# Martinsos/edlib

Measured on AMD Instinct MI355X. Metric: GCUPS (cell updates/s), 1M x 150bp HW reads vs 5Mb target, higher is better.
Workload: dtype u32

## Files before the change

edlib_amd/csrc/engine.hpp:

```cpp
#pragma once
#include "../../include/edlib_amd.h"
#include "common.hpp"
#include "pair_kernels.hpp"
#include "lanepair.hpp"
#include "reads_kernels.hpp"
#include "cross_kernels.hpp"
#include "window_kernels.hpp"
#include "strands.hpp"
#include "flat_pairs_prepare.hpp"
#include "pairs_gather.hpp"

#include <chrono>
#include <deque>
#include <functional>
#include <memory>
#include <vector>

namespace edlib_amd {

struct Tables {
    uint8_t tlut[256];
    uint8_t idToByte[256];
    int sigmaT = 0;
    uint32_t presence[8];
// ... 155 lines not shown
    std::vector<EdlibEqualityPair> eqs_;
    int device_ = 0;
    bool shared_ = false;
    bool pairsKind_ = false;
    bool noPairs_ = false;
    int noResults(const char* who);
    int n_ = 0;
    std::vector<long long> qoff_, toff_;
    bool strands_ = false;
    PinBuf h_strand_;
    int outN() const { return strands_ ? n_ / 2 : n_; }
    int unitOf(int u) const { return strands_ ? 2 * u + h_strand_.p[u] : u; }
    void setStrand(int read, int code) { h_strand_.p[read] = (uint8_t)(code & kStrandReverse); h_strand_.p[outN() + read] = (code & kStrandBoth) ? 1 : 0; }
    int resolveStrandsOnHost(std::vector<UnitResult>& res);
    int hostStrandCounts_[4] = {0, 0, 0, 0};
    int strandCounts(int counts[4]);
    Tables tab_;
    hipStream_t stream_ = nullptr;
    Event evRun0_, evRun1_, evA_, evB_;

    DevBuf<uint8_t> d_in_;
    PinBuf h_in_;
    DevBuf<uint8_t> d_qpool_, d_tpool_, d_tlut_, d_idToByte_, d_eq8_;
    DevBuf<uint16_t> d_eqtbl_;
    hipError_t uploadEq8();
    DevBuf<uint32_t> d_presence_;
    DevBuf<long long> d_qoff_, d_toff_;

    std::vector<int> emptyUnits_, readUnits_, pairUnits_;
    std::vector<int> longUnits_;
    std::vector<int> pairNow_;
    int beginRun(hipError_t guardStatus);
    int enqueueWordSteps();
    int endRun();
    void resetRecords(std::vector<UnitResult>& res);
    void answerEmptyUnits(std::vector<UnitResult>& res);
    int runFlatPhase(std::vector<UnitResult>& res, Lap& lap);
    int runLongReads(std::vector<UnitResult>& res, Lap& lap);
    int runPairPhase(std::vector<UnitResult>& res, Lap& lap);
    int runStartsPhase(std::vector<UnitResult>& res, Lap& lap);
    int runPathsPhase(std::vector<UnitResult>& res, Lap& lap);
    void startStats();
    bool flatDone_ = false;

    struct ReadGroup {
        int nwords = 0, nslots = 0, numSegments = 1, segLen = 0, warm = 0, mMin = 0, mMax = 0;
        std::vector<int> perm;
        DevBuf<int> d_perm, d_qlen, d_kinit, d_alphaExtra, d_segBest, d_segCnt, d_segPos;
        DevBuf<int> d_best, d_total, d_pos, d_flags;
        DevBuf<uint32_t> d_peq;
        bool zeroCopy = false; PinBuf hostOut;
        std::vector<int> ovfSlots; std::vector<long long> ovfOff; DevBuf<int> d_ovfPool;
        DevBuf<int> d_lvMap, d_lvBest, d_lvCnt, d_lvPos; std::vector<int> lvMap; int lvS = 0, lvCap = 0; bool lvValid = false;
        DevBuf<int> d_list;
        int nreal = -1;
        bool mates = false; DevBuf<int> d_win;
    };
    static constexpr int kLastLevelCap = 16;
    int listOpenSlots(ReadGroup& g, int kDone, std::vector<int>& out);
    DevBuf<uint8_t> d_selTmp_;
    std::vector<std::unique_ptr<ReadGroup>> groups_;
    DevBuf<uint32_t> d_tpk_, d_trows_;
    DevBuf<unsigned long long> d_wordSteps_;
    PinBuf h_wordSteps_; bool wordStepsPending_ = false;
    DevBuf<unsigned long long> d_ringSteps_; PinBuf h_ringSteps_; bool ringStepsUsed_ = false;
    unsigned long long* ringStepsCounter();
    bool banded_ = false;
    int syms_ = 4;
    int packTarget();
    int runReads();
    int makeGroup(const std::vector<int>& units, int words, std::unique_ptr<ReadGroup>& g, long long oneRoundWaves = 0);
    int runGroupScans(ReadGroup& g, bool fullOnly);
    int runGroupExact(ReadGroup& g);
    int collectGroup(ReadGroup& g, std::vector<UnitResult>& res);
    int seedThreshold(const ReadGroup& g, bool fullOnly) const;
    int buildSeedIndex();
    int runSeedPass(ReadGroup& g, int k);
    DevBuf<uint32_t> d_seedCnt_, d_seedOff_, d_seedPos_;
    DevBuf<uint8_t> d_seedTmp_;
    bool hits_ = false, hitsHaveRun_ = false;
    HitListBuffers hitList_;
    HitRows hostHits_;
    DevBuf<int> d_hitSlotUnit_;
    DevBuf<long long> d_hitTotal_;
    int runReadHits();
    int scanGroupHits(ReadGroup& g, int slotBase);
    int hitsScanBanded(ReadGroup& g, int slotBase, const int* d_slotmap, int nlanes, int numSegments, int segLen, int warm);
    struct Piece { long long off; int len; int thr; };
    int scanPieces(const std::vector<Piece>& pieces, bool filter, std::vector<std::pair<int, int>>* cand,
                   std::vector<uint8_t>* overflow, std::vector<int>* best);
    int solveLongReads(std::vector<UnitResult>& res, std::vector<int>& fallback);
    bool filterScan_ = false;
    struct ChainArgs { const uint32_t* in = nullptr; uint32_t* out = nullptr; const int* src = nullptr; int inLanes = 0, blocks = 0; const int* rowBase = nullptr; };
    ChainArgs chain_;
    int solveTallFull(const std::vector<int>& units, std::vector<UnitResult>& res, std::vector<int>& handBack);
    int collectReads(std::vector<UnitResult>& res);
    bool readsCollected_ = true;
    int scanGroup(ReadGroup& g, int mode, const int* d_slotmap, int nlanes, int kcap, const int* d_kinit,
                  int numSegments, int segLen, int warm, int* segBest, int* segCnt, int* segPos, int cap,
                  const long long* posOff, const int* posCap, bool unbanded = false,
                  unsigned long long* wordSteps = nullptr, const uint32_t* peqDense = nullptr,
                  const int* qlenDense = nullptr, int peqBottom = 0, int* liveBest = nullptr,
                  const Segment* segTable = nullptr, long long tableCols = 0);

    DevBuf<PairDesc> d_descs_;
    DevBuf<unsigned long long> d_peq64_;
// ... 201 lines not shown
```

edlib_amd/csrc/engine_reads.hip:

```cpp
#include "engine.hpp"

#include <algorithm>
#include <chrono>
#include <cmath>
#include <condition_variable>
#include <cstring>
#include <mutex>
#include <thread>

namespace edlib_amd {

__global__ void __launch_bounds__(256)
seed_thresholds_kernel(int* __restrict__ kinit, const int* __restrict__ best, const int* __restrict__ cnt, int n)
{
    const int i = blockIdx.x * blockDim.x + threadIdx.x;
    if (i < n && cnt[i] > 0 && best[i] < kinit[i]) kinit[i] = best[i];
}


int Batch::scanGroup(ReadGroup& g, int mode, const int* d_slotmap, int nlanes, int kcap, const int* d_kinit,
                     int numSegments, int segLen, int warm, int* segBest, int* segCnt, int* segPos, int cap,
                     const long long* posOff, const int* posCap, bool unbanded, unsigned long long* wordSteps,
                     const uint32_t* peqDense, const int* qlenDense, int peqBottom, int* liveBest,
                     const Segment* segTable, long long tableCols)
{
    ReadScanArgs a{};
    a.peq = peqDense ? peqDense : g.d_peq.p; a.tpk = d_tpk_.p; a.trows = d_trows_.p; a.targetLength = tlen(0);
    if (mode == EDLIB_MODE_SHW) a.targetLength = (int)std::min<long long>(a.targetLength, 64LL * g.nwords + 1);
    a.qlen = qlenDense ? qlenDense : g.d_qlen.p; a.kinit = d_kinit; a.slotmap = d_slotmap; a.nlanes = nlanes;
    a.numSegments = numSegments; a.segLen = segLen; a.warm = warm;
    a.segBest = segBest; a.segCnt = segCnt; a.segPos = segPos; a.cap = cap;
    a.posOff = posOff; a.posCap = posCap;
    a.kcap = kcap; a.wordSteps = wordSteps ? wordSteps : d_wordSteps_.p;
    a.filter = filterScan_ ? 1 : 0;
    a.liveBest = liveBest;
    a.segTable = segTable;
    a.bottomAligned = peqBottom;
    a.chainIn = chain_.in; a.chainOut = chain_.out; a.chainSrc = chain_.src; a.chainInLanes = chain_.inLanes;
    a.chainBlocks = chain_.blocks; a.rowBase = chain_.rowBase;
    const bool chained = chain_.in != nullptr || chain_.out != nullptr;
    const bool longGroup = g.nwords > kMaxReadWords;
    const bool fullHeight = banded_ && mode == EDLIB_MODE_HW && unbanded && (chained || syms_ > 4 || longGroup);
    const bool bandedKernel = !fullHeight && banded_ && mode == EDLIB_MODE_HW && (!unbanded || syms_ > 4 || longGroup);
    static const bool dbg = getenv("EDLIB_AMD_DEBUG") != nullptr;
    if (dbg) {
        EDLIB_AMD_HIP(hipStreamSynchronize(stream_));
        fprintf(stderr, "[edlib_amd] scanGroup nwords=%d mode=%d nlanes=%d S=%d segLen=%d warm=%d cap=%d kcap=%d slotmap=%p posOff=%p rows=%s kernel=%s syms=%d\n",
                g.nwords, mode, nlanes, numSegments, segLen, warm, cap, kcap, (const void*)d_slotmap, (const void*)posOff,
                peqBottom > 1 ? "delay" : (peqBottom ? "bottom" : "top"),
                fullHeight ? "full" : (bandedKernel ? "banded" : "plain"), syms_);
        if (peqBottom > 1) fprintf(stderr, "[edlib_amd] scanGroup delayRows=%d\n", peqBottom - 1);
    }
    scanTimerStart();
    const long long colsScanned = segTable ? tableCols
        : std::min<long long>(a.targetLength, (long long)numSegments * segLen) + (long long)(numSegments - 1) * warm;
#ifdef EDLIB_AMD_DRAIN_DIAG
    const char* drainOut = (peqBottom && liveBest) ? "edlib_amd_drain.bin" : nullptr;
    DevBuf<unsigned long long> d_clk;
    const size_t drainGX = ((size_t)(nlanes + 63) / 64 + 3) / 4, drainWaves = drainGX * numSegments * 4;
    if (drainOut) {
        EDLIB_AMD_HIP(d_clk.alloc(2 * drainWaves));
        EDLIB_AMD_HIP(hipMemsetAsync(d_clk.p, 0, 2 * drainWaves * sizeof(unsigned long long), stream_));
        a.waveClock = d_clk.p;
    }
#endif
    if (peqBottom && (fullHeight || bandedKernel)) EDLIB_AMD_HIP(hipErrorInvalidValue);
    if (fullHeight) {
        EDLIB_AMD_HIP(launch_scan_reads_full(g.nwords, syms_, a, stream_));
        stats.word_steps += (long long)((nlanes + 63) / 64 * 64) * g.nwords * colsScanned;
// ... 131 lines not shown
        }
        if (resolved > 0) {
            int acc = 0, kq = kFirstMax;
            for (int d = 0; d <= kFirstMax; ++d) { acc += hist[d]; if (acc * 1000LL >= resolved * 995LL) { kq = d; break; } }
            kFirst = std::max(4, std::min(kFirstMax, kq));
        }
        if (real > 0 && resolved * 10 < real * 3) twoPass = false;
        if (twoPass && (int)open.size() * 10 > real && open.size() >= 32 && price_ladder(open, open.size(), real)) return 1;
    }
    std::vector<int> todo;
    bool haveTodo = false;
    if (kSeed >= 0) {
        if (runSeedPass(g, kFirst)) return 1;
        if (twoPass) {
            if (listOpenSlots(g, kFirst, todo)) return 1;
            haveTodo = true;
            if (g.nreal < 0) { g.nreal = 0; for (int u : g.perm) g.nreal += u >= 0; }
            if (g.nslots >= 16384 && todo.size() * 10 > (size_t)g.nreal && todo.size() >= 32) {
                const size_t nsm = std::min<size_t>(2048, todo.size());
                std::vector<int> sample(nsm);
                for (size_t i = 0; i < nsm; ++i) sample[i] = todo[i * todo.size() / nsm];
                if (price_ladder(sample, todo.size(), g.nreal)) return 1;
            }
        }
    } else {
        if (scanGroup(g, mode, nullptr, g.nslots, twoPass ? kFirst : kNoCap, g.d_kinit.p, g.numSegments, g.segLen,
                      g.warm, g.d_segBest.p, g.d_segCnt.p, g.d_segPos.p, 8, nullptr, nullptr, fullOnly)) return 1;
        const bool chained = chain_.in != nullptr || chain_.out != nullptr;
        EDLIB_AMD_HIP(launch_merge_segments(g.d_segBest.p, g.d_segCnt.p, g.d_segPos.p, g.numSegments, 8,
                                            g.nslots, nullptr, 16, g.d_best.p, g.d_total.p, g.d_pos.p,
                                            g.d_flags.p, stream_, chained ? kOvfRescan : kOvfGatherGroup));
    }
    ladder.push_back(kNoCap);
    int kDone = kFirst;
    for (size_t lv = 0; twoPass && lv < ladder.size(); ++lv) {
        const int kcapL = ladder[lv];
        const bool last = kcapL == kNoCap;
        if (!haveTodo && listOpenSlots(g, kDone, todo)) return 1;
        haveTodo = false;
        if (todo.empty()) break;
        {
            const size_t no = todo.size();
            int S2, segLen2, warm2;
            plan_segments((int)no, T, mode, g.warm, 65536, S2, segLen2, warm2);
            const int capL = last ? kLastLevelCap : 8;
            EDLIB_AMD_HIP(g.d_lvMap.ensure(no));
            int* d_map = g.d_lvMap.p;
            EDLIB_AMD_HIP(hipMemcpyAsync(d_map, todo.data(), no * sizeof(int), hipMemcpyHostToDevice, stream_));
            bool plain = false;
            if (last && no >= 4096) {
                const int np2 = 64;
                std::vector<int> sub(np2);
                for (int i = 0; i < np2; ++i) sub[i] = todo[(size_t)((long long)i * no / np2)];
                int S3, segLen3, warm3;
                plan_segments(np2, T, mode, g.warm, 16384, S3, segLen3, warm3);
                const size_t it3 = (size_t)np2 * S3;
                DevBuf<int> d_m3, d_b3, d_c3, d_p3; DevBuf<unsigned long long> d_ws;
                EDLIB_AMD_HIP(d_m3.alloc(np2)); EDLIB_AMD_HIP(d_b3.alloc(it3)); EDLIB_AMD_HIP(d_c3.alloc(it3));
                EDLIB_AMD_HIP(d_p3.alloc(it3 * 8)); EDLIB_AMD_HIP(d_ws.alloc(1));
                EDLIB_AMD_HIP(hipMemcpyAsync(d_m3.p, sub.data(), np2 * sizeof(int), hipMemcpyHostToDevice, stream_));
                EDLIB_AMD_HIP(hipMemsetAsync(d_ws.p, 0, sizeof(unsigned long long), stream_));
                if (scanGroup(g, mode, d_m3.p, np2, kNoCap, g.d_kinit.p, S3, segLen3, warm3,
                              d_b3.p, d_c3.p, d_p3.p, 8, nullptr, nullptr, false, d_ws.p)) return 1;
                unsigned long long ws = 0;
                EDLIB_AMD_HIP(hipMemcpyAsync(&ws, d_ws.p, sizeof ws, hipMemcpyDeviceToHost, stream_));
                EDLIB_AMD_HIP(hipStreamSynchronize(stream_));
                const double cols = (double)np2 * ((double)T + (double)(S3 - 1) * warm3);
                plain = (double)ws >= 0.85 * g.nwords * cols;
                stats.word_steps += (long long)ws;
            }
            const bool bottomOk = plain && mode == EDLIB_MODE_HW && syms_ == 4 && g.nwords <= kMaxReadWords &&
                                  chain_.in == nullptr && chain_.out == nullptr;
            const int bottom = !bottomOk ? 0 : 1 + delay_rows_for(g.nwords, g.mMax);
            std::vector<Segment> table;
            DevBuf<Segment> d_segTable; long long tableCols = 0;
            if (bottom && S2 > 1 && no >= 4096) {
                int resident = 0;
                EDLIB_AMD_HIP(scan_reads_resident_workgroups(g.nwords, bottom, &resident));
#ifdef EDLIB_AMD_DRAIN_UNIFORM
                resident = 0;
#endif
                table = plan_segments_tapered(T, (int)(((no + 63) / 64 + 3) / 4), resident, warm2, segLen2);
                S2 = (int)table.size();
                for (const Segment& sg : table) tableCols += sg.cols + std::min(warm2, sg.start);
                EDLIB_AMD_HIP(d_segTable.alloc(table.size()));
                EDLIB_AMD_HIP(hipMemcpyAsync(d_segTable.p, table.data(), table.size() * sizeof(Segment), hipMemcpyHostToDevice, stream_));
            }
            const size_t items = no * (size_t)S2;
            EDLIB_AMD_HIP(g.d_lvBest.ensure(items)); EDLIB_AMD_HIP(g.d_lvCnt.ensure(items));
            EDLIB_AMD_HIP(g.d_lvPos.ensure(items * capL));
            int *d_sb = g.d_lvBest.p, *d_sc = g.d_lvCnt.p, *d_sp = g.d_lvPos.p;
            const size_t no64 = (no + 63) / 64 * 64;
            std::vector<int> perm2(no64, -1);
            for (size_t i = 0; i < no; ++i) perm2[i] = g.perm[todo[i]];
            DevBuf<int> d_perm2, d_qlen2, d_kinit2, d_extra2; DevBuf<uint32_t> d_peq2;
            EDLIB_AMD_HIP(d_perm2.alloc(no64)); EDLIB_AMD_HIP(d_qlen2.alloc(no64)); EDLIB_AMD_HIP(d_kinit2.alloc(no64));
            EDLIB_AMD_HIP(d_extra2.alloc(no64)); EDLIB_AMD_HIP(d_peq2.alloc(no64 * (size_t)syms_ * g.nwords));
            EDLIB_AMD_HIP(hipMemcpyAsync(d_perm2.p, perm2.data(), no64 * sizeof(int), hipMemcpyHostToDevice, stream_));
            EDLIB_AMD_HIP(launch_build_peq_reads(g.nwords, syms_, d_qpool_.p, d_qoff_.p, d_perm2.p, (int)no64,
                                                 d_eqtbl_.p, d_presence_.p, cfg_.k, d_peq2.p, d_qlen2.p,
                                                 d_kinit2.p, d_extra2.p, stream_, bottom));
            const int seedCols = 4096;
            DevBuf<int> d_b0, d_c0, d_p0;
            if (mode == EDLIB_MODE_HW && last && no >= 4096 && S2 > 1 && T >= 16 * seedCols) {
                EDLIB_AMD_HIP(d_b0.alloc(no)); EDLIB_AMD_HIP(d_c0.alloc(no)); EDLIB_AMD_HIP(d_p0.alloc(no * 8));
                if (scanGroup(g, mode, nullptr, (int)no, kcapL, d_kinit2.p, 1, seedCols, 0,
                              d_b0.p, d_c0.p, d_p0.p, 8, nullptr, nullptr, plain, nullptr, d_peq2.p, d_qlen2.p, bottom)) return 1;
                hipLaunchKernelGGL(seed_thresholds_kernel, dim3((unsigned)((no + 255) / 256)), dim3(256), 0, stream_,
                                   d_kinit2.p, d_b0.p, d_c0.p, (int)no);
                EDLIB_AMD_HIP(hipGetLastError());
            }
            DevBuf<int> d_live2;
            if (bottom && S2 > 1) {
                EDLIB_AMD_HIP(d_live2.alloc(no64));
                EDLIB_AMD_HIP(hipMemcpyAsync(d_live2.p, d_kinit2.p, no64 * sizeof(int), hipMemcpyDeviceToDevice, stream_));
            }
            if (scanGroup(g, mode, nullptr, (int)no, kcapL, d_kinit2.p, S2, segLen2, warm2,
                          d_sb, d_sc, d_sp, capL, nullptr, nullptr, plain, nullptr, d_peq2.p, d_qlen2.p, bottom, d_live2.p,
                          d_segTable.p, tableCols)) return 1;
            EDLIB_AMD_HIP(launch_merge_segments(d_sb, d_sc, d_sp, S2, capL, (int)no, d_map, 16,
                                                g.d_best.p, g.d_total.p, g.d_pos.p, g.d_flags.p, stream_,
                                                last ? kOvfGatherLevel : kOvfRescan));
            EDLIB_AMD_HIP(hipStreamSynchronize(stream_));
            if (last) { g.lvValid = true; g.lvS = S2; g.lvCap = capL; g.lvMap.swap(todo); }
            if (dbgLadder) fprintf(stderr, "[edlib_amd] level kcap=%d: %zu slots rescanned (plain=%d)\n", kcapL, no, (int)plain);
        }
        kDone = kcapL;
    }
    return 0;
}

int Batch::listOpenSlots(ReadGroup& g, int kDone, std::vector<int>& out)
{
    size_t tmp = 0;
    EDLIB_AMD_HIP(select_slots_scratch_bytes(g.nslots, &tmp));
    EDLIB_AMD_HIP(d_selTmp_.ensure(tmp));
    EDLIB_AMD_HIP(g.d_list.ensure((size_t)g.nslots + 1));
    int* count = g.d_list.p + g.nslots;
    EDLIB_AMD_HIP(launch_select_open_slots(g.d_perm.p, g.d_total.p, g.d_qlen.p, cfg_.k, kDone, g.nslots, g.d_list.p, count,
                                           d_selTmp_.p, d_selTmp_.bytes(), stream_, g.mates));
    int n = 0;
    EDLIB_AMD_HIP(hipMemcpyAsync(&n, count, sizeof(int), hipMemcpyDeviceToHost, stream_));
    EDLIB_AMD_HIP(hipStreamSynchronize(stream_));
    out.resize((size_t)n);
    if (n > 0) {
        EDLIB_AMD_HIP(hipMemcpyAsync(out.data(), g.d_list.p, (size_t)n * sizeof(int), hipMemcpyDeviceToHost, stream_));
        EDLIB_AMD_HIP(hipStreamSynchronize(stream_));
    }
    return 0;
}


int Batch::seedThreshold(const ReadGroup& g, bool fullOnly) const
{
    const long long T = tlen(0);
    if (fullOnly || !banded_ || cfg_.mode != EDLIB_MODE_HW || syms_ != 4 || cfg_.additionalEqualitiesLength > 0 ||
        g.nwords > kMaxReadWords || chain_.in != nullptr || chain_.out != nullptr)
        return -1;
    if (T < 64LL * 32 * g.nwords || g.nslots < 1024 || (long long)g.nslots * T < (1LL << 30)) return -1;
    int kf = -1;
    for (int k = 16; k >= 0 && kf < 0; --k) {
        const int L = g.mMin / (k + 1);
        if (L >= kSeedQ && (double)(k + 1) * (double)T <= std::ldexp(1.0, 2 * L) / 8.0) kf = k;
    }
    return (kf >= 0 && kf >= std::min(8, cfg_.k >= 0 ? cfg_.k : 8)) ? kf : -1;
}

int Batch::buildSeedIndex()
{
    const int T = tlen(0);
    EDLIB_AMD_HIP(d_seedCnt_.ensure((size_t)kSeedBuckets + 1));
    EDLIB_AMD_HIP(d_seedOff_.ensure((size_t)kSeedBuckets + 1));
    EDLIB_AMD_HIP(d_seedPos_.ensure((size_t)T));
    size_t tmp = 0;
    EDLIB_AMD_HIP(seed_index_scratch_bytes(&tmp));
    EDLIB_AMD_HIP(d_seedTmp_.ensure(tmp));
    scanTimerStart();
// ... 24 lines not shown
    static const bool dbg = getenv("EDLIB_AMD_DEBUG") != nullptr;
    if (dbg) fprintf(stderr, "[edlib_amd] seed pass nwords=%d k=%d: %d of %d slots handed back\n", g.nwords, k, nb, g.nslots);
    if (nb <= 0) return 0;
    int S2, segLen2, warm2;
    plan_segments(nb, T, EDLIB_MODE_HW, g.warm, 65536, S2, segLen2, warm2);
    const size_t items = (size_t)nb * S2;
    DevBuf<int> d_sb, d_sc, d_sp;
    EDLIB_AMD_HIP(d_sb.alloc(items)); EDLIB_AMD_HIP(d_sc.alloc(items)); EDLIB_AMD_HIP(d_sp.alloc(items * 8));
    if (scanGroup(g, EDLIB_MODE_HW, d_back.p, nb, k, g.d_kinit.p, S2, segLen2, warm2, d_sb.p, d_sc.p, d_sp.p, 8,
                  nullptr, nullptr)) return 1;
    EDLIB_AMD_HIP(launch_merge_segments(d_sb.p, d_sc.p, d_sp.p, S2, 8, nb, d_back.p, 16, g.d_best.p, g.d_total.p,
                                        g.d_pos.p, g.d_flags.p, stream_));
    EDLIB_AMD_HIP(hipStreamSynchronize(stream_));
    return 0;
}

int Batch::runGroupExact(ReadGroup& g)
{
    const int T = tlen(0);
    const int mode = (cfg_.mode == EDLIB_MODE_HW || cfg_.mode == EDLIB_MODE_SHW) ? (int)cfg_.mode : (int)EDLIB_MODE_NW;
    const int kNoCap = 0x3fffffff;
    const size_t ns = (size_t)g.nslots;
    g.ovfSlots.clear(); g.ovfOff.assign(1, 0);
    if (mode == EDLIB_MODE_NW) return 0;
    std::vector<int> recs;
    if (g.zeroCopy && !g.mates) {
        EDLIB_AMD_HIP(hipStreamSynchronize(stream_));
        for (size_t s = 0; s < ns; ++s)
            if (g.d_flags.p[s] && g.perm[s] >= 0) { recs.push_back((int)s); recs.push_back(g.d_flags.p[s]); recs.push_back(g.d_total.p[s]); }
    } else {
        size_t tmp = 0;
        EDLIB_AMD_HIP(select_slots_scratch_bytes(g.nslots, &tmp));
        EDLIB_AMD_HIP(d_selTmp_.ensure(tmp));
        EDLIB_AMD_HIP(g.d_list.ensure(ns + 1));
        int* count = g.d_list.p + ns;
        EDLIB_AMD_HIP(launch_select_flagged_slots(g.d_perm.p, g.d_flags.p, g.nslots, g.d_list.p, count,
                                                  d_selTmp_.p, d_selTmp_.bytes(), stream_, g.mates ? g.d_win.p : nullptr));
        int novf = 0;
        EDLIB_AMD_HIP(hipMemcpyAsync(&novf, count, sizeof(int), hipMemcpyDeviceToHost, stream_));
        EDLIB_AMD_HIP(hipStreamSynchronize(stream_));
        if (novf > 0) {
            DevBuf<int> d_recs;
            EDLIB_AMD_HIP(d_recs.alloc((size_t)novf * 3));
            EDLIB_AMD_HIP(launch_pick_slot_records(g.d_list.p, novf, g.d_flags.p, g.d_total.p, d_recs.p, stream_));
            recs.resize((size_t)novf * 3);
            EDLIB_AMD_HIP(hipMemcpyAsync(recs.data(), d_recs.p, recs.size() * sizeof(int), hipMemcpyDeviceToHost, stream_));
            EDLIB_AMD_HIP(hipStreamSynchronize(stream_));
        }
    }
    const size_t no = recs.size() / 3;
    if (!no) return 0;
    std::vector<int> src(no, 0), at(no, -1);
    std::vector<int> rescan;
    for (size_t i = 0; i < no; ++i) {
        const int s = recs[3 * i], f = recs[3 * i + 1];
        g.ovfSlots.push_back(s);
        if (f == kOvfGatherLevel && g.lvValid) {
            const auto it = std::lower_bound(g.lvMap.begin(), g.lvMap.end(), s);
            if (it != g.lvMap.end() && *it == s) { src[i] = 1; at[i] = (int)(it - g.lvMap.begin()); }
        } else if (f == kOvfGatherGroup) { src[i] = 2; at[i] = s; }
        if (!src[i]) { at[i] = (int)rescan.size(); rescan.push_back(s); }
    }
    const size_t nr = rescan.size();
    int S2 = 1, segLen2 = 0, warm2 = 0;
    DevBuf<int> d_map, d_caps, d_sb, d_sc; DevBuf<long long> d_off;
    std::vector<int> cnts;
    if (nr) {
        plan_segments((int)nr, T, mode, g.warm, 16384, S2, segLen2, warm2, nr <= 256 ? 1024 : 4096);
        const size_t items = nr * (size_t)S2;
        EDLIB_AMD_HIP(d_map.alloc(nr)); EDLIB_AMD_HIP(d_sb.alloc(items)); EDLIB_AMD_HIP(d_sc.alloc(items));
        EDLIB_AMD_HIP(hipMemcpyAsync(d_map.p, rescan.data(), nr * sizeof(int), hipMemcpyHostToDevice, stream_));
        if (scanGroup(g, mode, d_map.p, (int)nr, kNoCap, g.d_best.p, S2, segLen2, warm2,
                      d_sb.p, d_sc.p, d_sb.p , 0, nullptr, nullptr)) return 1;
        cnts.resize(items);
        EDLIB_AMD_HIP(hipMemcpyAsync(cnts.data(), d_sc.p, items * sizeof(int), hipMemcpyDeviceToHost, stream_));
        EDLIB_AMD_HIP(hipStreamSynchronize(stream_));
    }
    std::vector<long long> offs(nr * (size_t)S2);
    std::vector<int> gIdx[2], gLim[2]; std::vector<long long> gOff[2];
    long long acc = 0;
    g.ovfOff.assign(no + 1, 0);
    for (size_t i = 0; i < no; ++i) {
        if (src[i]) {
            const int w = src[i] - 1, n = std::max(0, recs[3 * i + 2]);
            gIdx[w].push_back(at[i]); gOff[w].push_back(acc); gLim[w].push_back(n);
            acc += n;
        } else {
            const size_t r = (size_t)at[i];
            for (int sg = 0; sg < S2; ++sg) { offs[r * S2 + sg] = acc; acc += cnts[r * S2 + sg]; }
        }
        g.ovfOff[i + 1] = acc;
    }
    EDLIB_AMD_HIP(g.d_ovfPool.ensure((size_t)std::max<long long>(acc, 1)));
    DevBuf<int> d_gi[2], d_gl[2]; DevBuf<long long> d_go[2];
    for (int w = 0; w < 2; ++w) {
        const size_t n = gIdx[w].size();
        if (!n) continue;
        EDLIB_AMD_HIP(d_gi[w].alloc(n)); EDLIB_AMD_HIP(d_gl[w].alloc(n)); EDLIB_AMD_HIP(d_go[w].alloc(n));
        EDLIB_AMD_HIP(hipMemcpyAsync(d_gi[w].p, gIdx[w].data(), n * sizeof(int), hipMemcpyHostToDevice, stream_));
        EDLIB_AMD_HIP(hipMemcpyAsync(d_gl[w].p, gLim[w].data(), n * sizeof(int), hipMemcpyHostToDevice, stream_));
        EDLIB_AMD_HIP(hipMemcpyAsync(d_go[w].p, gOff[w].data(), n * sizeof(long long), hipMemcpyHostToDevice, stream_));
        if (w == 0)
            EDLIB_AMD_HIP(launch_gather_segments(g.d_lvBest.p, g.d_lvCnt.p, g.d_lvPos.p, g.lvS, g.lvCap, (int)n,
                                                 d_gi[w].p, d_go[w].p, d_gl[w].p, g.d_ovfPool.p, stream_));
        else
            EDLIB_AMD_HIP(launch_gather_segments(g.d_segBest.p, g.d_segCnt.p, g.d_segPos.p, g.numSegments, 8, (int)n,
                                                 d_gi[w].p, d_go[w].p, d_gl[w].p, g.d_ovfPool.p, stream_));
    }
    if (nr) {
        const size_t items = nr * (size_t)S2;
        EDLIB_AMD_HIP(d_caps.alloc(items)); EDLIB_AMD_HIP(d_off.alloc(items));
        EDLIB_AMD_HIP(hipMemcpyAsync(d_caps.p, cnts.data(), items * sizeof(int), hipMemcpyHostToDevice, stream_));
        EDLIB_AMD_HIP(hipMemcpyAsync(d_off.p, offs.data(), items * sizeof(long long), hipMemcpyHostToDevice, stream_));
        if (scanGroup(g, mode, d_map.p, (int)nr, kNoCap, g.d_best.p, S2, segLen2, warm2,
                      d_sb.p, d_sc.p, g.d_ovfPool.p, 0, d_off.p, d_caps.p)) return 1;
    }
    EDLIB_AMD_HIP(hipStreamSynchronize(stream_));
    static const bool dbg = getenv("EDLIB_AMD_DEBUG") != nullptr;
    if (dbg) fprintf(stderr, "[edlib_amd] exact pass nwords=%d: %zu gathered, %zu rescanned\n", g.nwords, no - nr, nr);
    stats.overflow_units += (int)no;
    return 0;
}


int Batch::hitsScanBanded(ReadGroup& g, int slotBase, const int* d_slotmap, int nlanes, int numSegments, int segLen, int warm)
{
    ReadScanArgs a{};
    a.peq = g.d_peq.p; a.tpk = d_tpk_.p; a.trows = d_trows_.p; a.targetLength = tlen(0);
    a.qlen = g.d_qlen.p; a.kinit = g.d_kinit.p; a.slotmap = d_slotmap; a.nlanes = nlanes;
    a.numSegments = numSegments; a.segLen = segLen; a.warm = warm;
    a.cap = 1;
    a.kcap = 0x3fffffff; a.wordSteps = d_wordSteps_.p;
    a.hits = hitList_.list(); a.slotBase = slotBase;
    scanTimerStart();
    EDLIB_AMD_HIP(launch_scan_reads_hits(g.nwords, syms_, a, stream_));
    scanTimerStop();
    return 0;
}

int Batch::scanGroupHits(ReadGroup& g, int slotBase)
{
    const int T = tlen(0);
    const int kSeed = seedThreshold(g, false);
    if (kSeed < 0 || cfg_.k > kSeed) return hitsScanBanded(g, slotBase, nullptr, g.nslots, g.numSegments, g.segLen, g.warm);
    DevBuf<int> d_back;
    EDLIB_AMD_HIP(d_back.alloc((size_t)g.nslots + 1));
    int* backCount = d_back.p + g.nslots;
    EDLIB_AMD_HIP(hipMemsetAsync(backCount, 0, sizeof(int), stream_));
    SeedArgs a{};
    a.peq = g.d_peq.p; a.qlen = g.d_qlen.p; a.perm = g.d_perm.p; a.tpk = d_tpk_.p; a.targetLength = T;
    a.seedOff = d_seedOff_.p; a.seedPos = d_seedPos_.p; a.nslots = g.nslots; a.k = cfg_.k;
    a.backSlots = d_back.p; a.backCount = backCount; a.wordSteps = d_wordSteps_.p;
    a.hits = hitList_.list(); a.slotBase = slotBase;
    scanTimerStart();
    EDLIB_AMD_HIP(launch_seed_verify_hits(g.nwords, a, stream_));
    scanTimerStop();
    int nb = 0;
    EDLIB_AMD_HIP(hipMemcpyAsync(&nb, backCount, sizeof(int), hipMemcpyDeviceToHost, stream_));
    EDLIB_AMD_HIP(hipStreamSynchronize(stream_));
    static const bool dbg = getenv("EDLIB_AMD_DEBUG") != nullptr;
    if (dbg) fprintf(stderr, "[edlib_amd] seed hits pass nwords=%d k=%d: %d of %d slots handed back\n", g.nwords, cfg_.k, nb, g.nslots);
    if (nb > 0) {
        int S2, segLen2, warm2;
        plan_segments(nb, T, EDLIB_MODE_HW, g.warm, 65536, S2, segLen2, warm2);
        if (hitsScanBanded(g, slotBase, d_back.p, nb, S2, segLen2, warm2)) return 1;
        EDLIB_AMD_HIP(hipStreamSynchronize(stream_));
    }
    return 0;
}

int Batch::runReadHits()
{
// ... 149 lines not shown
```

edlib_amd/csrc/reads_kernels.hip:

```cpp
#include "reads_kernels.hpp"
#include "reads_scan.hpp"
#include "reads_column_asm.hpp"

namespace edlib_amd {


__global__ void __launch_bounds__(256)
pack_target_2bit_kernel(const uint8_t* __restrict__ raw, const uint8_t* __restrict__ lut,
                        int T, u32* __restrict__ tpk, int nwords)
{
    __shared__ uint8_t s_lut[256];
    s_lut[threadIdx.x] = lut[threadIdx.x];
    __syncthreads();
    const int w = blockIdx.x * blockDim.x + threadIdx.x;
    if (w >= nwords) return;
    const int base = w * 16;
    u32 out = 0;
    if (base + 16 <= T) {
        const uint4 v = *reinterpret_cast<const uint4*>(raw + base);
        const u32 d[4] = {v.x, v.y, v.z, v.w};
#pragma unroll
        for (int i = 0; i < 16; ++i)
            out |= (u32)(s_lut[(d[i >> 2] >> ((i & 3) * 8)) & 0xFF] & 3) << (2 * i);
    } else {
// ... 568 lines not shown
}

hipError_t launch_merge_segments(const int* segBest, const int* segCnt, const int* segPos, int S,
                                 int cap, int nlanes, const int* slotmap, int capFinal, int* best,
                                 int* total, int* pos, int* flags, hipStream_t stream, int gatherFlag)
{
    if (nlanes == 0) return hipSuccess;
    if (S >= 64) {
        hipLaunchKernelGGL(merge_segments_wave_kernel, dim3(nlanes), dim3(64), 0, stream,
                           segBest, segCnt, segPos, S, cap, nlanes, slotmap, capFinal, best, total, pos, flags, gatherFlag);
        return hipGetLastError();
    }
    hipLaunchKernelGGL(merge_segments_kernel, dim3((nlanes + 255) / 256), dim3(256), 0, stream,
                       segBest, segCnt, segPos, S, cap, nlanes, slotmap, capFinal, best, total, pos, flags, gatherFlag);
    return hipGetLastError();
}

__global__ void __launch_bounds__(64)
gather_segments_kernel(const int* __restrict__ segBest, const int* __restrict__ segCnt,
                       const int* __restrict__ segPos, int S, int cap, const int* __restrict__ idx,
                       const long long* __restrict__ off, const int* __restrict__ lim, int* __restrict__ out)
{
    const int lane = threadIdx.x;
    const size_t base = (size_t)idx[blockIdx.x] * S;
    int* dst = out + off[blockIdx.x];
    const int capOut = lim[blockIdx.x];
    int b = 0x7fffffff;
    for (int s = lane; s < S; s += 64)
        if (segCnt[base + s] > 0 && segBest[base + s] < b) b = segBest[base + s];
    for (int o = 32; o; o >>= 1) { const int t = __shfl_xor(b, o); b = t < b ? t : b; }
    if (b == 0x7fffffff) return;
    int n = 0;
    for (int s0 = 0; s0 < S; s0 += 64) {
        const int s = s0 + lane;
        int c = s < S ? segCnt[base + s] : 0;
        if (c <= 0 || segBest[base + s] != b) c = 0;
        int incl = c;
        for (int d = 1; d < 64; d <<= 1) { const int t = __shfl_up(incl, d); if (lane >= d) incl += t; }
        const int at = n + incl - c, take = c < cap ? c : cap;
        for (int i = 0; i < take; ++i)
            if (at + i < capOut) dst[at + i] = segPos[(base + s) * cap + i];
        n += __shfl(incl, 63);
    }
}

hipError_t launch_gather_segments(const int* segBest, const int* segCnt, const int* segPos, int S, int cap, int n,
                                  const int* idx, const long long* off, const int* lim, int* out, hipStream_t stream)
{
    if (n == 0) return hipSuccess;
    hipLaunchKernelGGL(gather_segments_kernel, dim3(n), dim3(64), 0, stream, segBest, segCnt, segPos, S, cap, idx, off, lim, out);
    return hipGetLastError();
}

}
```

edlib_amd/csrc/reads_kernels.hpp:

```cpp
#pragma once
#include <hip/hip_runtime.h>
#include <stdint.h>

#include "hit_list.hpp"
#include "segment_plan.hpp"

namespace edlib_amd {

constexpr int kMaxReadWords = 8;
constexpr int kMaxLongReadWords = 16;
constexpr int kMaxLongReadWords4 = 32;
constexpr int kFilterFromWords = 13;
inline int read_group_words(int m) { const int w = (m + 31) / 32; return w <= kMaxReadWords ? w : (w <= 10 ? 10 : (w <= 12 ? 12 : (w <= 14 ? 14 : (w <= 16 ? 16 : (w <= 24 ? 24 : 32))))); }
constexpr int kDelayRowsDeep = 7, kDelayRowsShallow = 3;
constexpr bool delay_rows_fit(int nwords, int longest, int rows) { return nwords <= kMaxReadWords && longest >= 1 && longest + rows <= 32 * nwords; }
constexpr int delay_rows_for(int nwords, int longest)
{
    return delay_rows_fit(nwords, longest, kDelayRowsDeep) ? kDelayRowsDeep : (delay_rows_fit(nwords, longest, kDelayRowsShallow) ? kDelayRowsShallow : 0);
}
constexpr bool bottom_align_valid(int b) { return b == 0 || b == 1 || b == 1 + kDelayRowsShallow || b == 1 + kDelayRowsDeep; }
constexpr int kLanes = 64;


struct ReadScanArgs {
// ... 38 lines not shown

hipError_t launch_scan_reads_banded(int nwords, int syms, const ReadScanArgs& a, hipStream_t stream);

hipError_t launch_scan_reads_full(int nwords, int syms, const ReadScanArgs& a, hipStream_t stream);

hipError_t launch_pack_target_2bit(const uint8_t* raw, const uint8_t* lut, int targetLength,
                                   uint32_t* tpk, hipStream_t stream);
hipError_t launch_pack_target_rows(const uint8_t* raw, const uint8_t* lut, int targetLength,
                                   uint32_t* trows, int ndwords, hipStream_t stream);

hipError_t launch_build_peq_reads(int nwords, int syms, const uint8_t* reads, const long long* qoff,
                                  const int* perm, int nslots, const uint16_t* eqtbl,
                                  const uint32_t* targetPresence , int kcfg,
                                  uint32_t* peq, int* qlen, int* kinit, int* alphaExtra,
                                  hipStream_t stream, int bottomAlign = 0);

hipError_t launch_collect_candidates(const int* segCnt, const int* segPos, int numSegments, int cap, int nlanes,
                                     int* out, int maxOut, int* counter, int* overflow, hipStream_t stream);

constexpr int kSeedQ = 12;
constexpr int kSeedBuckets = 1 << (2 * kSeedQ);
constexpr int kSeedBucketCap = 64;
constexpr int kSeedMaxDiag = 32;
constexpr int kSeedMaxWindow = 1024;

struct SeedArgs {
    const uint32_t* peq;
    const int* qlen;
    const int* perm;
    const uint32_t* tpk;
    int targetLength;
    const uint32_t* seedOff;
    const uint32_t* seedPos;
    int nslots;
    int k;
    int* best; int* total; int* pos; int* flags;
    int* backSlots; int* backCount;
    unsigned long long* wordSteps;
    HitList hits;
    int slotBase;
};

hipError_t seed_index_scratch_bytes(size_t* bytes);
hipError_t launch_build_seed_index(const uint32_t* tpk, int targetLength, uint32_t* cnt, uint32_t* off, uint32_t* pos,
                                   void* tmp, size_t tmpBytes, hipStream_t stream);
hipError_t launch_seed_verify(int nwords, const SeedArgs& a, hipStream_t stream);

hipError_t launch_merge_segments(const int* segBest, const int* segCnt, const int* segPos,
                                 int numSegments, int cap, int nlanes, const int* slotmap, int capFinal,
                                 int* best, int* total, int* pos, int* flags, hipStream_t stream, int gatherFlag = 1);
constexpr int kOvfRescan = 1, kOvfGatherLevel = 2, kOvfGatherGroup = 4;
hipError_t launch_gather_segments(const int* segBest, const int* segCnt, const int* segPos, int numSegments, int cap, int n,
                                  const int* idx, const long long* off, const int* lim, int* out, hipStream_t stream);

hipError_t select_slots_scratch_bytes(int nslots, size_t* bytes);
hipError_t launch_select_open_slots(const int* perm, const int* total, const int* qlen, int kcfg, int kDone, int nslots,
                                    int* out, int* count, void* tmp, size_t tmpBytes, hipStream_t stream, bool mates = false);
hipError_t launch_select_flagged_slots(const int* perm, const int* flags, int nslots, int* out, int* count,
                                       void* tmp, size_t tmpBytes, hipStream_t stream, const int* win = nullptr);
hipError_t launch_pick_slot_records(const int* slots, int n, const int* flags, const int* total, int* out, hipStream_t stream);

hipError_t launch_scan_reads_hits(int nwords, int syms, const ReadScanArgs& a, hipStream_t stream);
hipError_t launch_seed_verify_hits(int nwords, const SeedArgs& a, hipStream_t stream);
constexpr int kReadHitsExtraBytes = 12;
hipError_t launch_read_hits_finish(HitListBuffers& hl, const int* slotUnit, int numUnits, long long* total, hipStream_t stream);

}
```

Baseline: 3.458 million.

## Rescan overflowed reads only in overflowing segments and segment the seed pass

Overflowed reads from the last ladder level are now re-scanned only over the segments that overflowed, split into sub-segments. Positions from segments that did not overflow are copied on device instead of re-scanning the whole target. The band-share census uses fixed-size segments without position output. The seed-threshold pre-pass is split into multiple segments to expose more parallelism, and the per-level permutation is gathered on device instead of built on the host. This adds host syncs and device-to-host copies of per-segment counts, plus more bookkeeping complexity.

Result: no change. 3.489 million, median of 6 (+0.9%).

```diff
diff --git a/edlib_amd/csrc/engine.hpp b/edlib_amd/csrc/engine.hpp
--- a/edlib_amd/csrc/engine.hpp
+++ b/edlib_amd/csrc/engine.hpp
@@ -231,6 +231,7 @@
         bool zeroCopy = false; PinBuf hostOut;
         std::vector<int> ovfSlots; std::vector<long long> ovfOff; DevBuf<int> d_ovfPool;
         DevBuf<int> d_lvMap, d_lvBest, d_lvCnt, d_lvPos; std::vector<int> lvMap; int lvS = 0, lvCap = 0; bool lvValid = false;
+        std::vector<Segment> lvTable;
         DevBuf<int> d_list;
         int nreal = -1;
         bool mates = false; DevBuf<int> d_win;
diff --git a/edlib_amd/csrc/engine_reads.hip b/edlib_amd/csrc/engine_reads.hip
--- a/edlib_amd/csrc/engine_reads.hip
+++ b/edlib_amd/csrc/engine_reads.hip
@@ -11,10 +11,14 @@
 namespace edlib_amd {
 
 __global__ void __launch_bounds__(256)
-seed_thresholds_kernel(int* __restrict__ kinit, const int* __restrict__ best, const int* __restrict__ cnt, int n)
+seed_thresholds_kernel(int* __restrict__ kinit, const int* __restrict__ best, const int* __restrict__ cnt, int n, int S)
 {
     const int i = blockIdx.x * blockDim.x + threadIdx.x;
-    if (i < n && cnt[i] > 0 && best[i] < kinit[i]) kinit[i] = best[i];
+    if (i >= n) return;
+    int b = kinit[i];
+    for (int s = 0; s < S; ++s)
+        if (cnt[(size_t)i * S + s] > 0 && best[(size_t)i * S + s] < b) b = best[(size_t)i * S + s];
+    kinit[i] = b;
 }
 
 
@@ -252,22 +256,30 @@
                 const int np2 = 64;
                 std::vector<int> sub(np2);
                 for (int i = 0; i < np2; ++i) sub[i] = todo[(size_t)((long long)i * no / np2)];
-                int S3, segLen3, warm3;
-                plan_segments(np2, T, mode, g.warm, 16384, S3, segLen3, warm3);
-                const size_t it3 = (size_t)np2 * S3;
-                DevBuf<int> d_m3, d_b3, d_c3, d_p3; DevBuf<unsigned long long> d_ws;
-                EDLIB_AMD_HIP(d_m3.alloc(np2)); EDLIB_AMD_HIP(d_b3.alloc(it3)); EDLIB_AMD_HIP(d_c3.alloc(it3));
-                EDLIB_AMD_HIP(d_p3.alloc(it3 * 8)); EDLIB_AMD_HIP(d_ws.alloc(1));
+                DevBuf<int> d_m3;
+                EDLIB_AMD_HIP(d_m3.alloc(np2));
                 EDLIB_AMD_HIP(hipMemcpyAsync(d_m3.p, sub.data(), np2 * sizeof(int), hipMemcpyHostToDevice, stream_));
-                EDLIB_AMD_HIP(hipMemsetAsync(d_ws.p, 0, sizeof(unsigned long long), stream_));
-                if (scanGroup(g, mode, d_m3.p, np2, kNoCap, g.d_kinit.p, S3, segLen3, warm3,
-                              d_b3.p, d_c3.p, d_p3.p, 8, nullptr, nullptr, false, d_ws.p)) return 1;
-                unsigned long long ws = 0;
-                EDLIB_AMD_HIP(hipMemcpyAsync(&ws, d_ws.p, sizeof ws, hipMemcpyDeviceToHost, stream_));
-                EDLIB_AMD_HIP(hipStreamSynchronize(stream_));
-                const double cols = (double)np2 * ((double)T + (double)(S3 - 1) * warm3);
-                plain = (double)ws >= 0.85 * g.nwords * cols;
+                auto band_share = [&](int S3, int segLen3, int warm3, double& share, unsigned long long& ws) -> int {
+                    const size_t it3 = (size_t)np2 * S3;
+                    DevBuf<int> d_b3, d_c3; DevBuf<unsigned long long> d_ws;
+                    EDLIB_AMD_HIP(d_b3.alloc(it3)); EDLIB_AMD_HIP(d_c3.alloc(it3)); EDLIB_AMD_HIP(d_ws.alloc(1));
+                    EDLIB_AMD_HIP(hipMemsetAsync(d_ws.p, 0, sizeof(unsigned long long), stream_));
+                    if (scanGroup(g, mode, d_m3.p, np2, kNoCap, g.d_kinit.p, S3, segLen3, warm3,
+                                  d_b3.p, d_c3.p, d_b3.p , 0, nullptr, nullptr, false, d_ws.p)) return 1;
+                    EDLIB_AMD_HIP(hipMemcpyAsync(&ws, d_ws.p, sizeof ws, hipMemcpyDeviceToHost, stream_));
+                    EDLIB_AMD_HIP(hipStreamSynchronize(stream_));
+                    const double cols = (double)np2 * ((double)std::min<long long>(T, (long long)S3 * segLen3) + (double)(S3 - 1) * warm3);
+                    share = (double)ws / (g.nwords * cols);
+                    return 0;
+                };
+                const int warm3 = g.warm, segLen3 = seg_roundup16(std::max(1024LL, 4LL * g.warm));
+                const int S3 = (int)std::min<long long>(2048, std::max<long long>(1, ((long long)T + segLen3 - 1) / segLen3));
+                double share = 0.0; unsigned long long ws = 0;
+                if (band_share(S3, segLen3, warm3, share, ws)) return 1;
+                plain = share >= 0.85;
                 stats.word_steps += (long long)ws;
+                if (dbgLadder)
+                    fprintf(stderr, "[edlib_amd] census nwords=%d: band share %.4f over %d segments of %d columns\n", g.nwords, share, S3, segLen3);
             }
             const bool bottomOk = plain && mode == EDLIB_MODE_HW && syms_ == 4 && g.nwords <= kMaxReadWords &&
                                   chain_.in == nullptr && chain_.out == nullptr;
@@ -291,23 +303,24 @@
             EDLIB_AMD_HIP(g.d_lvPos.ensure(items * capL));
             int *d_sb = g.d_lvBest.p, *d_sc = g.d_lvCnt.p, *d_sp = g.d_lvPos.p;
             const size_t no64 = (no + 63) / 64 * 64;
-            std::vector<int> perm2(no64, -1);
-            for (size_t i = 0; i < no; ++i) perm2[i] = g.perm[todo[i]];
             DevBuf<int> d_perm2, d_qlen2, d_kinit2, d_extra2; DevBuf<uint32_t> d_peq2;
             EDLIB_AMD_HIP(d_perm2.alloc(no64)); EDLIB_AMD_HIP(d_qlen2.alloc(no64)); EDLIB_AMD_HIP(d_kinit2.alloc(no64));
             EDLIB_AMD_HIP(d_extra2.alloc(no64)); EDLIB_AMD_HIP(d_peq2.alloc(no64 * (size_t)syms_ * g.nwords));
-            EDLIB_AMD_HIP(hipMemcpyAsync(d_perm2.p, perm2.data(), no64 * sizeof(int), hipMemcpyHostToDevice, stream_));
+            EDLIB_AMD_HIP(launch_gather_perm(g.d_perm.p, d_map, (int)no, (int)no64, d_perm2.p, stream_));
             EDLIB_AMD_HIP(launch_build_peq_reads(g.nwords, syms_, d_qpool_.p, d_qoff_.p, d_perm2.p, (int)no64,
                                                  d_eqtbl_.p, d_presence_.p, cfg_.k, d_peq2.p, d_qlen2.p,
                                                  d_kinit2.p, d_extra2.p, stream_, bottom));
             const int seedCols = 4096;
-            DevBuf<int> d_b0, d_c0, d_p0;
+            DevBuf<int> d_b0, d_c0;
             if (mode == EDLIB_MODE_HW && last && no >= 4096 && S2 > 1 && T >= 16 * seedCols) {
-                EDLIB_AMD_HIP(d_b0.alloc(no)); EDLIB_AMD_HIP(d_c0.alloc(no)); EDLIB_AMD_HIP(d_p0.alloc(no * 8));
-                if (scanGroup(g, mode, nullptr, (int)no, kcapL, d_kinit2.p, 1, seedCols, 0,
-                              d_b0.p, d_c0.p, d_p0.p, 8, nullptr, nullptr, plain, nullptr, d_peq2.p, d_qlen2.p, bottom)) return 1;
+                int S0, segLen0, warm0;
+                plan_segments_uniform((int)no, seedCols, true, g.warm, 2 * 1024, 1024, S0, segLen0, warm0);
+                if ((long long)((no + 63) / 64) * S0 < 2 * 1024) { S0 = 1; segLen0 = seedCols; warm0 = 0; }
+                EDLIB_AMD_HIP(d_b0.alloc(no * (size_t)S0)); EDLIB_AMD_HIP(d_c0.alloc(no * (size_t)S0));
+                if (scanGroup(g, mode, nullptr, (int)no, kcapL, d_kinit2.p, S0, segLen0, warm0,
+                              d_b0.p, d_c0.p, d_b0.p , 0, nullptr, nullptr, plain, nullptr, d_peq2.p, d_qlen2.p, bottom)) return 1;
                 hipLaunchKernelGGL(seed_thresholds_kernel, dim3((unsigned)((no + 255) / 256)), dim3(256), 0, stream_,
-                                   d_kinit2.p, d_b0.p, d_c0.p, (int)no);
+                                   d_kinit2.p, d_b0.p, d_c0.p, (int)no, S0);
                 EDLIB_AMD_HIP(hipGetLastError());
             }
             DevBuf<int> d_live2;
@@ -322,7 +335,10 @@
                                                 g.d_best.p, g.d_total.p, g.d_pos.p, g.d_flags.p, stream_,
                                                 last ? kOvfGatherLevel : kOvfRescan));
             EDLIB_AMD_HIP(hipStreamSynchronize(stream_));
-            if (last) { g.lvValid = true; g.lvS = S2; g.lvCap = capL; g.lvMap.swap(todo); }
+            if (last) {
+                g.lvValid = true; g.lvS = S2; g.lvCap = capL; g.lvMap.swap(todo);
+                if (table.empty()) g.lvTable = uniform_segment_table(T, segLen2); else g.lvTable.swap(table);
+            }
             if (dbgLadder) fprintf(stderr, "[edlib_amd] level kcap=%d: %zu slots rescanned (plain=%d)\n", kcapL, no, (int)plain);
         }
         kDone = kcapL;
@@ -453,16 +469,43 @@
     if (!no) return 0;
     std::vector<int> src(no, 0), at(no, -1);
     std::vector<int> rescan;
+    const bool chained = chain_.in != nullptr || chain_.out != nullptr;
+    const bool bySegment = g.lvValid && mode == EDLIB_MODE_HW && syms_ == 4 && g.nwords <= kMaxReadWords && !chained &&
+                           g.lvS > 0 && g.lvTable.size() == (size_t)g.lvS;
+    const size_t lvS = (size_t)std::max(g.lvS, 0);
+    std::vector<int> once, onceLane, lvCntH, lvBestH;
     for (size_t i = 0; i < no; ++i) {
         const int s = recs[3 * i], f = recs[3 * i + 1];
         g.ovfSlots.push_back(s);
-        if (f == kOvfGatherLevel && g.lvValid) {
+        if ((f == kOvfGatherLevel || (f == kOvfRescan && bySegment)) && g.lvValid) {
             const auto it = std::lower_bound(g.lvMap.begin(), g.lvMap.end(), s);
-            if (it != g.lvMap.end() && *it == s) { src[i] = 1; at[i] = (int)(it - g.lvMap.begin()); }
+            if (it != g.lvMap.end() && *it == s) {
+                src[i] = f == kOvfGatherLevel ? 1 : 3; at[i] = (int)(it - g.lvMap.begin());
+                if (src[i] == 3) { once.push_back((int)i); onceLane.push_back(at[i]); }
+            }
         } else if (f == kOvfGatherGroup) { src[i] = 2; at[i] = s; }
-        if (!src[i]) { at[i] = (int)rescan.size(); rescan.push_back(s); }
-    }
-    const size_t nr = rescan.size();
+    }
+    std::vector<char> parent(lvS, 0);
+    if (!once.empty()) {
+        lvCntH.resize(once.size() * lvS); lvBestH.resize(once.size() * lvS);
+        for (size_t r = 0; r < once.size(); ++r) {
+            EDLIB_AMD_HIP(hipMemcpyAsync(&lvCntH[r * lvS], g.d_lvCnt.p + (size_t)onceLane[r] * lvS, lvS * sizeof(int), hipMemcpyDeviceToHost, stream_));
+            EDLIB_AMD_HIP(hipMemcpyAsync(&lvBestH[r * lvS], g.d_lvBest.p + (size_t)onceLane[r] * lvS, lvS * sizeof(int), hipMemcpyDeviceToHost, stream_));
+        }
+        EDLIB_AMD_HIP(hipStreamSynchronize(stream_));
+        for (size_t r = 0; r < once.size(); ++r) {
+            int* c = &lvCntH[r * lvS]; const int* b = &lvBestH[r * lvS];
+            int bb = 0x7fffffff;
+            for (size_t sg = 0; sg < lvS; ++sg) if (c[sg] > 0 && b[sg] < bb) bb = b[sg];
+            for (size_t sg = 0; sg < lvS; ++sg) {
+                if (c[sg] <= 0 || b[sg] != bb) c[sg] = 0;
+                if (c[sg] > g.lvCap) parent[sg] = 1;
+            }
+        }
+    }
+    for (size_t i = 0; i < no; ++i)
+        if (!src[i]) { at[i] = (int)rescan.size(); rescan.push_back(recs[3 * i]); }
+    const size_t nr = rescan.size(), nr1 = once.size();
     int S2 = 1, segLen2 = 0, warm2 = 0;
     DevBuf<int> d_map, d_caps, d_sb, d_sc; DevBuf<long long> d_off;
     std::vector<int> cnts;
@@ -479,10 +522,36 @@
     }
     std::vector<long long> offs(nr * (size_t)S2);
     std::vector<int> gIdx[2], gLim[2]; std::vector<long long> gOff[2];
+    std::vector<Segment> subs; std::vector<int2> subOf(lvS, int2{0, 0});
+    std::vector<long long> dst1(nr1 * lvS, -1);
+    if (nr1) {
+        long long pcols = 0;
+        for (size_t sg = 0; sg < lvS; ++sg) if (parent[sg]) pcols += g.lvTable[sg].cols;
+        int subLen = 1024;
+        while (pcols / subLen + (long long)lvS > kMaxSegments) subLen *= 2;
+        for (size_t sg = 0; sg < lvS; ++sg) {
+            if (!parent[sg]) continue;
+            subOf[sg].x = (int)subs.size();
+            const int end = g.lvTable[sg].start + g.lvTable[sg].cols;
+            for (int c = g.lvTable[sg].start; c < end; ) {
+                const int len = end - c < subLen + subLen / 4 ? end - c : subLen;
+                subs.push_back({c, len});
+                c += len;
+            }
+            subOf[sg].y = (int)subs.size();
+        }
+    }
     long long acc = 0;
+    size_t r1 = 0;
     g.ovfOff.assign(no + 1, 0);
     for (size_t i = 0; i < no; ++i) {
-        if (src[i]) {
+        if (src[i] == 3) {
+            for (size_t sg = 0; sg < lvS; ++sg) {
+                const int c = lvCntH[r1 * lvS + sg];
+                if (c > 0) { dst1[r1 * lvS + sg] = acc; acc += c; }
+            }
+            ++r1;
+        } else if (src[i]) {
             const int w = src[i] - 1, n = std::max(0, recs[3 * i + 2]);
             gIdx[w].push_back(at[i]); gOff[w].push_back(acc); gLim[w].push_back(n);
             acc += n;
@@ -516,9 +585,61 @@
         if (scanGroup(g, mode, d_map.p, (int)nr, kNoCap, g.d_best.p, S2, segLen2, warm2,
                       d_sb.p, d_sc.p, g.d_ovfPool.p, 0, d_off.p, d_caps.p)) return 1;
     }
+    DevBuf<int> d_map1, d_lane1, d_sb1, d_sc1, d_cap1; DevBuf<long long> d_off1, d_dst1; DevBuf<Segment> d_subTable;
+    std::vector<int> map1, cap1, cnt1; std::vector<long long> off1, copy1;
+    if (nr1) {
+        const size_t NS = subs.size(), items = nr1 * NS;
+        map1.resize(nr1); cap1.assign(items, 0); off1.assign(items, 0); cnt1.assign(items, 0);
+        long long tableCols = 0;
+        for (const Segment& sg : subs) tableCols += sg.cols + std::min(g.warm, sg.start);
+        for (size_t r = 0; r < nr1; ++r) map1[r] = recs[3 * (size_t)once[r]];
+        EDLIB_AMD_HIP(d_map1.alloc(nr1)); EDLIB_AMD_HIP(d_lane1.alloc(nr1)); EDLIB_AMD_HIP(d_sb1.alloc(items)); EDLIB_AMD_HIP(d_sc1.alloc(items));
+        EDLIB_AMD_HIP(d_cap1.alloc(items)); EDLIB_AMD_HIP(d_off1.alloc(items)); EDLIB_AMD_HIP(d_dst1.alloc(nr1 * lvS));
+        EDLIB_AMD_HIP(d_subTable.alloc(NS));
+        EDLIB_AMD_HIP(hipMemcpyAsync(d_map1.p, map1.data(), nr1 * sizeof(int), hipMemcpyHostToDevice, stream_));
+        EDLIB_AMD_HIP(hipMemcpyAsync(d_lane1.p, onceLane.data(), nr1 * sizeof(int), hipMemcpyHostToDevice, stream_));
+        EDLIB_AMD_HIP(hipMemcpyAsync(d_subTable.p, subs.data(), NS * sizeof(Segment), hipMemcpyHostToDevice, stream_));
+        if (NS) {
+            if (scanGroup(g, mode, d_map1.p, (int)nr1, kNoCap, g.d_best.p, (int)NS, 1024, g.warm,
+                          d_sb1.p, d_sc1.p, d_sb1.p , 0, nullptr, nullptr, true, nullptr, nullptr, nullptr, 0, nullptr,
+                          d_subTable.p, tableCols)) return 1;
+            EDLIB_AMD_HIP(hipMemcpyAsync(cnt1.data(), d_sc1.p, items * sizeof(int), hipMemcpyDeviceToHost, stream_));
+            EDLIB_AMD_HIP(hipStreamSynchronize(stream_));
+        }
+        copy1 = dst1;
+        for (size_t r = 0; r < nr1; ++r)
+            for (size_t sg = 0; sg < lvS; ++sg) {
+                const int c = lvCntH[r * lvS + sg];
+                if (c <= g.lvCap) continue;
+                copy1[r * lvS + sg] = -1;
+                int n = 0;
+                for (int j = subOf[sg].x; j < subOf[sg].y; ++j) {
+                    off1[r * NS + j] = dst1[r * lvS + sg] + n;
+                    cap1[r * NS + j] = std::max(0, std::min(cnt1[r * NS + j], c - n));
+                    n += cap1[r * NS + j];
+                }
+            }
+        EDLIB_AMD_HIP(hipMemcpyAsync(d_dst1.p, copy1.data(), nr1 * lvS * sizeof(long long), hipMemcpyHostToDevice, stream_));
+        EDLIB_AMD_HIP(launch_copy_level_segments(g.d_lvCnt.p, g.d_lvPos.p, g.lvS, g.lvCap, d_lane1.p, (int)nr1, d_dst1.p,
+                                                 g.d_ovfPool.p, stream_));
+        if (NS) {
+            EDLIB_AMD_HIP(hipMemcpyAsync(d_cap1.p, cap1.data(), items * sizeof(int), hipMemcpyHostToDevice, stream_));
+            EDLIB_AMD_HIP(hipMemcpyAsync(d_off1.p, off1.data(), items * sizeof(long long), hipMemcpyHostToDevice, stream_));
+            if (scanGroup(g, mode, d_map1.p, (int)nr1, kNoCap, g.d_best.p, (int)NS, 1024, g.warm,
+                          d_sb1.p, d_sc1.p, g.d_ovfPool.p, 0, d_off1.p, d_cap1.p, true, nullptr, nullptr, nullptr, 0, nullptr,
+                          d_subTable.p, tableCols)) return 1;
+        }
+    }
     EDLIB_AMD_HIP(hipStreamSynchronize(stream_));
     static const bool dbg = getenv("EDLIB_AMD_DEBUG") != nullptr;
-    if (dbg) fprintf(stderr, "[edlib_amd] exact pass nwords=%d: %zu gathered, %zu rescanned\n", g.nwords, no - nr, nr);
+    if (dbg) {
+        fprintf(stderr, "[edlib_amd] exact pass nwords=%d: %zu gathered, %zu rescanned\n", g.nwords, no - nr - nr1, nr + nr1);
+        fprintf(stderr, "[edlib_amd] exact pass nwords=%d: by segment (%zu sub-segments):", g.nwords, subs.size());
+        for (size_t r = 0; r < nr1; ++r) fprintf(stderr, " %d", g.perm[map1[r]]);
+        fprintf(stderr, "; whole target:");
+        for (int s : rescan) fprintf(stderr, " %d", g.perm[s]);
+        fprintf(stderr, "\n");
+    }
     stats.overflow_units += (int)no;
     return 0;
 }
diff --git a/edlib_amd/csrc/reads_kernels.hip b/edlib_amd/csrc/reads_kernels.hip
--- a/edlib_amd/csrc/reads_kernels.hip
+++ b/edlib_amd/csrc/reads_kernels.hip
@@ -644,4 +644,41 @@
     return hipGetLastError();
 }
 
-}
+__global__ void __launch_bounds__(256)
+copy_level_segments_kernel(const int* __restrict__ lvCnt, const int* __restrict__ lvPos, int S, int cap,
+                           const int* __restrict__ lanes, int nr, const long long* __restrict__ dst, int* __restrict__ out)
+{
+    const long long item = (long long)blockIdx.x * blockDim.x + threadIdx.x;
+    if (item >= (long long)nr * S) return;
+    const long long at = dst[item];
+    if (at < 0) return;
+    const size_t base = (size_t)lanes[item / S] * S + (size_t)(item % S);
+    const int c = lvCnt[base];
+    for (int i = 0; i < c && i < cap; ++i) out[at + i] = lvPos[base * cap + i];
+}
+
+hipError_t launch_copy_level_segments(const int* lvCnt, const int* lvPos, int S, int cap, const int* lanes, int nr,
+                                      const long long* dst, int* out, hipStream_t stream)
+{
+    const long long items = (long long)nr * S;
+    if (items == 0) return hipSuccess;
+    hipLaunchKernelGGL(copy_level_segments_kernel, dim3((unsigned)((items + 255) / 256)), dim3(256), 0, stream,
+                       lvCnt, lvPos, S, cap, lanes, nr, dst, out);
+    return hipGetLastError();
+}
+
+__global__ void __launch_bounds__(256)
+gather_perm_kernel(const int* __restrict__ perm, const int* __restrict__ map, int n, int nOut, int* __restrict__ out)
+{
+    const int i = blockIdx.x * blockDim.x + threadIdx.x;
+    if (i < nOut) out[i] = i < n ? perm[map[i]] : -1;
+}
+
+hipError_t launch_gather_perm(const int* perm, const int* map, int n, int nOut, int* out, hipStream_t stream)
+{
+    if (nOut == 0) return hipSuccess;
+    hipLaunchKernelGGL(gather_perm_kernel, dim3((unsigned)((nOut + 255) / 256)), dim3(256), 0, stream, perm, map, n, nOut, out);
+    return hipGetLastError();
+}
+
+}
diff --git a/edlib_amd/csrc/reads_kernels.hpp b/edlib_amd/csrc/reads_kernels.hpp
--- a/edlib_amd/csrc/reads_kernels.hpp
+++ b/edlib_amd/csrc/reads_kernels.hpp
@@ -114,6 +114,9 @@
 constexpr int kOvfRescan = 1, kOvfGatherLevel = 2, kOvfGatherGroup = 4;
 hipError_t launch_gather_segments(const int* segBest, const int* segCnt, const int* segPos, int numSegments, int cap, int n,
                                   const int* idx, const long long* off, const int* lim, int* out, hipStream_t stream);
+hipError_t launch_copy_level_segments(const int* lvCnt, const int* lvPos, int S, int cap, const int* lanes, int nr,
+                                      const long long* dst, int* out, hipStream_t stream);
+hipError_t launch_gather_perm(const int* perm, const int* map, int n, int nOut, int* out, hipStream_t stream);
 
 hipError_t select_slots_scratch_bytes(int nslots, size_t* bytes);
 hipError_t launch_select_open_slots(const int* perm, const int* total, const int* qlen, int kcfg, int kDone, int nslots,
```
